# pppKin/rs_ray_toy

Measured on NVIDIA B200. Metric: Mrays/s incoherent closest-hit, higher is better.
Workload: dtype f64 deciding arithmetic (Moller-Trumbore / quadratic), fp32 box culling

## Files before the change

rs_ray_toy_b200/csrc/aggregate.cu:

```cuda
#include <cuda_runtime.h>

#include <chrono>
#include <cmath>
#include <cstdio>
#include <cstdlib>
#include <algorithm>
#include <atomic>
#include <cstring>
#include <thread>
#include <vector>

#include "aggregate.hpp"
#include "bvh_lbvh.hpp"
#include "bvh_pack_plan.hpp"
#include "device_layout.h"
#include "sphere_core.cuh"
#include "tri_screen.h"

namespace rrt {

namespace {

constexpr int kStack = 64;
#ifndef RRT_BLOCK
// ... 140 lines not shown
        *prim_id = (uint32_t)__double2loint(r4.y);
        *kind = (uint32_t)__double2hiint(r4.y);
        *a = {r0.x, r0.y, r1.x};
        *b = {r1.y, r2.x, r2.y};
        *c = {r3.x, r3.y, r4.x};
    }
}

__device__ __noinline__ bool prepare_ray(const AggView& A, D3 o, D3 d, double t_max, float* t_shift, RayF* rf) {
    const double len2 = d.x * d.x + d.y * d.y + d.z * d.z;
    if (!(len2 > 0.0) || !(len2 < 1e300) || !(o.x == o.x) || !(o.y == o.y) || !(o.z == o.z) ||
        fabs(o.x) > 1e300 || fabs(o.y) > 1e300 || fabs(o.z) > 1e300)
        return false;
    double ts = 0.0;
    bool outside = o.x < A.world_lo[0] || o.x > A.world_hi[0] || o.y < A.world_lo[1] || o.y > A.world_hi[1] ||
                   o.z < A.world_lo[2] || o.z > A.world_hi[2];
    if (outside) {
        double t0 = 0.0, t1 = t_max;
        const double oo[3] = {o.x, o.y, o.z}, dd[3] = {d.x, d.y, d.z};
#pragma unroll
        for (int k = 0; k < 3; ++k) {
            if (dd[k] == 0.0) {
                if (oo[k] < A.world_lo[k] || oo[k] > A.world_hi[k]) return false;
                continue;
            }
            double inv = 1.0 / dd[k];
            double ta = (A.world_lo[k] - oo[k]) * inv, tb = (A.world_hi[k] - oo[k]) * inv;
            double tn = fmin(ta, tb), tf = fmax(ta, tb);
            tf *= 1.0 + 1e-12;
            t0 = fmax(t0, tn);
            t1 = fmin(t1, tf);
        }
        if (t0 > t1 * (1.0 + 1e-12) + 1e-300) return false;
        double len = sqrt(d.x * d.x + d.y * d.y + d.z * d.z);
        ts = fmax(0.0, t0 - A.scene_scale / len);
    }
    const float tsf = __double2float_rd(ts);
    ts = (double)tsf;
    *t_shift = tsf;
    double sx = o.x + d.x * ts, sy = o.y + d.y * ts, sz = o.z + d.z * ts;
    const float ix = safe_inv(d.x), iy = safe_inv(d.y), iz = safe_inv(d.z);
    if (A.quantised) {
        rf->idx = A.grid_ext[0] * ix;
        rf->idy = A.grid_ext[1] * iy;
        rf->idz = A.grid_ext[2] * iz;
        rf->oidx = (float)(sx - A.grid_c[0]) * ix;
        rf->oidy = (float)(sy - A.grid_c[1]) * iy;
        rf->oidz = (float)(sz - A.grid_c[2]) * iz;
    } else {
        rf->idx = ix;
        rf->idy = iy;
        rf->idz = iz;
        rf->oidx = (float)sx * ix;
        rf->oidy = (float)sy * iy;
        rf->oidz = (float)sz * iz;
    }
    return true;
}

__device__ __noinline__ bool general_sphere_test(const AggView& A, double index, D3 o, D3 d, double t_far, double* t) {
    const GenSphere& g = static_cast<const GenSphere*>(A.gspheres)[(uint32_t)index];
    V3 p;
    double phi;
    return gen_sphere_hit(g, v3(o.x, o.y, o.z), v3(d.x, d.y, d.z), t_far, t, &p, &phi);
}

template <bool WIDE>
__device__ __noinline__ void hit_params(const AggView& A, uint32_t rec, D3 o, D3 d, double t, double* u, double* v) {
    D3 a, b, c;
    uint32_t pid, kind, inst = 0xFFFFFFFFu;
    load_prim<WIDE>(A.prims, rec, &a, &b, &c, &pid, &kind);
    if (kind == PRIM_TRIANGLE) {
        double tt;
        tri_test(o, d, a, b, c, &tt, u, v);
        return;
    }
    if (kind == PRIM_SPHERE_GENERAL) {
        const GenSphere& g = static_cast<const GenSphere*>(A.gspheres)[(uint32_t)a.x];
        V3 p;
        double phi, tt;
        *u = *v = 0.0;
        if (gen_sphere_hit(g, v3(o.x, o.y, o.z), v3(d.x, d.y, d.z), t, &tt, &p, &phi)) gen_sphere_uv(g, p, phi, u, v);
        return;
    }
    if (!WIDE) inst = static_cast<const PrimRec48*>(A.prims)[rec].words[8];
    else inst = static_cast<const PrimRec96*>(A.prims)[rec].pad[0];
    D3 lo = o, ld = d;
    if (inst != 0xFFFFFFFFu) {
        const double* m = A.inst_w2p + 12 * (size_t)inst;
        lo = {__dadd_rn(__dadd_rn(__dadd_rn(__dmul_rn(m[0], o.x), __dmul_rn(m[1], o.y)), __dmul_rn(m[2], o.z)), m[3]),
              __dadd_rn(__dadd_rn(__dadd_rn(__dmul_rn(m[4], o.x), __dmul_rn(m[5], o.y)), __dmul_rn(m[6], o.z)), m[7]),
              __dadd_rn(__dadd_rn(__dadd_rn(__dmul_rn(m[8], o.x), __dmul_rn(m[9], o.y)), __dmul_rn(m[10], o.z)), m[11])};
        ld = {__dadd_rn(__dadd_rn(__dmul_rn(m[0], d.x), __dmul_rn(m[1], d.y)), __dmul_rn(m[2], d.z)),
              __dadd_rn(__dadd_rn(__dmul_rn(m[4], d.x), __dmul_rn(m[5], d.y)), __dmul_rn(m[6], d.z)),
              __dadd_rn(__dadd_rn(__dmul_rn(m[8], d.x), __dmul_rn(m[9], d.y)), __dmul_rn(m[10], d.z))};
    }
    const double radius = b.x;
    double px = __dadd_rn(lo.x, __dmul_rn(ld.x, t)), py = __dadd_rn(lo.y, __dmul_rn(ld.y, t)),
           pz = __dadd_rn(lo.z, __dmul_rn(ld.z, t));
    if (px == 0.0 && py == 0.0) px = __dmul_rn(1e-5, radius);
    double phi = atan2(py, px);
    const double kPi = 3.14159265358979323846;
    if (phi < 0.0) phi = __dadd_rn(phi, __dmul_rn(2.0, kPi));
    const double phi_max = __dmul_rn(360.0, kPi / 180.0);
    *u = __ddiv_rn(phi, phi_max);
    double cz = __ddiv_rn(pz, radius);
    cz = cz < -1.0 ? -1.0 : (cz > 1.0 ? 1.0 : cz);
    double theta = acos(cz);
    const double theta_min = kPi, theta_max = 0.0;
    *v = __ddiv_rn(__dsub_rn(theta, theta_min), __dsub_rn(theta_max, theta_min));
}

constexpr int32_t kDone = 0x7fffffff;
constexpr int32_t kNoLeaf = 0;
#ifndef RRT_REFILL
#define RRT_REFILL 8
#endif
#ifndef RRT_NODE32
#define RRT_NODE32 1
#endif
#ifndef RRT_STALE_SKIP
#define RRT_STALE_SKIP 0
#endif
#ifndef RRT_STATS
#define RRT_STATS 0
#endif
#ifndef RRT_WALK_MIN
#define RRT_WALK_MIN 12
#endif
#ifndef RRT_PREFETCH_FAR
#define RRT_PREFETCH_FAR 0
#endif
#ifndef RRT_LEAF_MIN
#define RRT_LEAF_MIN 8
#endif
#ifndef RRT_LEAF_TRIPS
#define RRT_LEAF_TRIPS 0
#endif
#ifndef RRT_LEAFQ
#define RRT_LEAFQ 3
#endif
#ifndef RRT_MINBLOCKS
#define RRT_MINBLOCKS 7
#endif
#ifndef RRT_MINBLOCKS_Q
#define RRT_MINBLOCKS_Q 8
#endif
#ifndef RRT_STAGE_TOP
#define RRT_STAGE_TOP 0
#endif
constexpr int kStageTop = RRT_STAGE_TOP;
constexpr int kRefill = RRT_REFILL;
constexpr int kScreenRows = RRT_PRETEST ? 9 : 0;


template <bool ANY, bool WIDE, bool QUANT, bool GEN>
__global__ void __launch_bounds__(kBlock, QUANT ? RRT_MINBLOCKS_Q : RRT_MINBLOCKS) trace_kernel(AggView A, uint64_t n, const rrt_ray* __restrict__ rays,
                                                        rrt_hit* __restrict__ hits, uint8_t* __restrict__ occluded,
                                                        const uint32_t* __restrict__ perm,
                                                        const uint32_t* __restrict__ use_perm,
                                                        unsigned long long* __restrict__ cursor,
                                                        const uint32_t* __restrict__ n_dev, int stack_levels) {
    const unsigned FULL = 0xffffffffu;
    if (n_dev) n = *n_dev;
    const unsigned lane = threadIdx.x & 31u;
    const Node64* __restrict__ nodes = static_cast<const Node64*>(A.nodes);
    const bool permuted = perm != nullptr && (use_perm == nullptr || *use_perm != 0u);

    extern __shared__ int32_t sstack[];
    int32_t* const my_stack = sstack + threadIdx.x;
#if RRT_STALE_SKIP
    float* const my_tstack = reinterpret_cast<float*>(sstack + stack_levels * kBlock) + threadIdx.x;
#define RRT_POP()                                                      \
    do {                                                               \
        --sp;                                                          \
        node = my_stack[sp * kBlock];                                  \
    } while (!ANY && my_tstack[sp * kBlock] > tcull)
#else
#define RRT_POP()                     \
    do {                              \
        --sp;                         \
        node = my_stack[sp * kBlock]; \
    } while (0)
#endif
    float* const my_screen = reinterpret_cast<float*>(sstack + stack_levels * kBlock * (RRT_STALE_SKIP ? 2 : 1)) + threadIdx.x;
#if RRT_STAGE_TOP
    uint4* const s_top = reinterpret_cast<uint4*>(sstack + (stack_levels * (RRT_STALE_SKIP ? 2 : 1) + kScreenRows) * kBlock);
    if (QUANT) {
        const uint4* src = static_cast<const uint4*>(A.nodes);
        const int n_stage = A.n_staged;
        for (int k = threadIdx.x; k < 2 * n_stage; k += kBlock) s_top[k] = __ldg(src + k);
        __syncthreads();
    }
#endif
    int sp = 1;
    int32_t node = kDone;
    int32_t leaf = kNoLeaf;
#if RRT_LEAFQ > 1
    int32_t lq[RRT_LEAFQ - 1];
#pragma unroll
    for (int k = 0; k < RRT_LEAFQ - 1; ++k) lq[k] = kNoLeaf;
#define RRT_PARK()                                         \
    do {                                                   \
        bool placed_ = false;                              \
        if (leaf == kNoLeaf) {                             \
            leaf = node;                                   \
            placed_ = true;                                \
        }                                                  \
        _Pragma("unroll") for (int k_ = 0; k_ < RRT_LEAFQ - 1; ++k_) { \
            if (!placed_ && lq[k_] == kNoLeaf) {           \
                lq[k_] = node;                             \
                placed_ = true;                            \
            }                                              \
        }                                                  \
    } while (0)
#endif
    bool have_ray = false;
    bool exhausted = false;
    uint64_t ray_index = 0;
    D3 o = {0, 0, 0}, d = {0, 0, 0};
    RayF rf = {0, 0, 0, 0, 0, 0};
    uint32_t selx = 0x4105u, sely = 0x4105u, selz = 0x4105u;
    double best_t = 0.0;
    float t_shift = 0.0f, tcull = 0.0f;
    uint32_t best_id = RRT_NO_HIT, best_rec = 0;
    bool found = false;
#if RRT_STATS
    unsigned long long st_trips = 0, st_walk = 0, st_noray = 0, st_drained = 0, st_second = 0, st_ltrips = 0, st_lact = 0;
#endif

    for (;;) {
        const bool finished = have_ray && node == kDone && leaf == kNoLeaf;
        if (finished) {
            if (ANY) {
                occluded[ray_index] = found ? 1 : 0;
            } else {
                double bu = 0.0, bv = 0.0;
                const bool got = best_id != RRT_NO_HIT;
                if (got) hit_params<WIDE>(A, best_rec, o, d, best_t, &bu, &bv);
                double2* hp = reinterpret_cast<double2*>(hits + ray_index);
                double2 w0, w1;
                w0.x = __hiloint2double(0, (int)best_id);
                w0.y = got ? best_t : 0.0;
                w1.x = bu;
                w1.y = bv;
                __stcs(hp, w0);
                __stcs(hp + 1, w1);
            }
            have_ray = false;
        }
        const unsigned idle = __ballot_sync(FULL, !have_ray);
        if (idle != 0u && !exhausted && (__popc(idle) >= kRefill)) {
            const int want = __popc(idle);
            unsigned long long base = 0;
            if (lane == 0) base = atomicAdd(cursor, (unsigned long long)want);
            base = __shfl_sync(FULL, base, 0);
            if (base + (unsigned long long)want >= n) exhausted = true;
            if (!have_ray) {
                const unsigned long long q = base + (unsigned long long)__popc(idle & ((1u << lane) - 1u));
                if (q < n) {
                    ray_index = permuted ? (uint64_t)__ldcs(perm + q) : (uint64_t)q;
                    const double2* rp = reinterpret_cast<const double2*>(rays + ray_index);
                    const double2 q0 = __ldcs(rp), q1 = __ldcs(rp + 1), q2 = __ldcs(rp + 2), q3 = __ldcs(rp + 3);
                    o = {q0.x, q0.y, q1.x};
                    d = {q1.y, q2.x, q2.y};
                    best_t = q3.x;
                    best_id = RRT_NO_HIT;
                    found = false;
                    have_ray = true;
                    sp = 1;
                    my_stack[0] = kDone;
#if RRT_STALE_SKIP
                    my_tstack[0] = -1.0f;
#endif
                    leaf = kNoLeaf;
#if RRT_LEAFQ > 1
#pragma unroll
                    for (int k = 0; k < RRT_LEAFQ - 1; ++k) lq[k] = kNoLeaf;
#endif
                    if (!WIDE && RRT_PRETEST) {
                        const ScreenRay R = make_screen_ray(o.x, o.y, o.z, d.x, d.y, d.z);
                        my_screen[0 * kBlock] = R.ox; my_screen[1 * kBlock] = R.oy; my_screen[2 * kBlock] = R.oz;
                        my_screen[3 * kBlock] = R.dx; my_screen[4 * kBlock] = R.dy; my_screen[5 * kBlock] = R.dz;
                        my_screen[6 * kBlock] = R.mo;
                        my_screen[7 * kBlock] = R.md;
                        my_screen[8 * kBlock] = R.kmd;
                    }
                    const bool live = prepare_ray(A, o, d, best_t, &t_shift, &rf) && !(best_t < 0.0);
                    node = live ? A.root : kDone;
                    tcull = __double2float_ru(best_t - (double)t_shift);
                    if (QUANT && RRT_SIGN_SELECT) {
                        selx = rf.idx < 0.0f ? 0x4325u : 0x4105u;
                        sely = rf.idy < 0.0f ? 0x4325u : 0x4105u;
                        selz = rf.idz < 0.0f ? 0x4325u : 0x4105u;
                    }
                }
            }
        }
        if (__ballot_sync(FULL, have_ray) == 0u) {
            if (exhausted) break;
            continue;
        }

        for (;;) {
#pragma unroll
          for (int step = 0; step < RRT_UNROLL; ++step) {
            const bool walking = node >= 0 && node != kDone;
#if RRT_STATS
            st_trips += 1;
            st_walk += __popc(__ballot_sync(FULL, walking));
            st_noray += __popc(__ballot_sync(FULL, !have_ray));
            st_drained += __popc(__ballot_sync(FULL, have_ray && node == kDone));
            st_second += __popc(__ballot_sync(FULL, have_ray && node < 0));
#endif
            if (walking) {
                int32_t ch_x, ch_y;
                float tn0, tn1;
                bool h0, h1;
                if (QUANT) {
#if RRT_STAGE_TOP
                    F8 v;
                    if (node < A.n_staged) {
                        const uint4 lo = s_top[2 * node], hi = s_top[2 * node + 1];
                        v = F8{__uint_as_float(lo.x), __uint_as_float(lo.y), __uint_as_float(lo.z), __uint_as_float(lo.w),
                               __uint_as_float(hi.x), __uint_as_float(hi.y), __uint_as_float(hi.z), __uint_as_float(hi.w)};
                    } else {
                        v = ldg256(reinterpret_cast<const char*>(A.nodes) + (size_t)node * sizeof(Node32));
                    }
#else
                    const F8 v = ldg256(reinterpret_cast<const char*>(A.nodes) + (size_t)node * sizeof(Node32));
#endif
                    const uint32_t w0 = __float_as_uint(v.a), w1 = __float_as_uint(v.b), w2 = __float_as_uint(v.c);
                    const uint32_t w3 = __float_as_uint(v.d), w4 = __float_as_uint(v.e), w5 = __float_as_uint(v.f);
                    ch_x = __float_as_int(v.g);
                    ch_y = __float_as_int(v.h);
#define RRT_QLO(w) __uint_as_float(__byte_perm((w), 0x3Fu, 0x4105))
#define RRT_QHI(w) __uint_as_float(__byte_perm((w), 0x3Fu, 0x4325))
#if RRT_SIGN_SELECT
                    h0 = slab_q(rf, w0, w1, w2, selx, sely, selz, tcull, &tn0);
                    h1 = slab_q(rf, w3, w4, w5, selx, sely, selz, tcull, &tn1);
#else
                    h0 = slab(rf, RRT_QLO(w0), RRT_QHI(w0), RRT_QLO(w1), RRT_QHI(w1), RRT_QLO(w2), RRT_QHI(w2), tcull, &tn0);
                    h1 = slab(rf, RRT_QLO(w3), RRT_QHI(w3), RRT_QLO(w4), RRT_QHI(w4), RRT_QLO(w5), RRT_QHI(w5), tcull, &tn1);
#endif
                } else {
                    const char* np = reinterpret_cast<const char*>(nodes + node);
                    const F8 lo = ldg256(np);
                    const F8 hi = ldg256(np + 32);
                    ch_x = __float_as_int(hi.e);
                    ch_y = __float_as_int(hi.f);
                    h0 = slab(rf, lo.a, lo.b, lo.c, lo.d, hi.a, hi.b, tcull, &tn0);
                    h1 = slab(rf, lo.e, lo.f, lo.g, lo.h, hi.c, hi.d, tcull, &tn1);
                }
                const bool both = h0 && h1;
                const bool swap = !ANY && (tn1 < tn0);
                const int32_t near_c = swap ? ch_y : ch_x, far_c = swap ? ch_x : ch_y;
                if (both) {
                    my_stack[sp * kBlock] = far_c;
#if RRT_PREFETCH_FAR
                    if (far_c >= 0) {
                        const char* fp = reinterpret_cast<const char*>(A.nodes) + (size_t)far_c * (QUANT ? sizeof(Node32) : sizeof(Node64));
#if RRT_PREFETCH_FAR == 1
                        asm volatile("prefetch.global.L2 [%0];" ::"l"(fp));
#else
                        asm volatile("prefetch.global.L1 [%0];" ::"l"(fp));
#endif
                    }
#endif
#if RRT_STALE_SKIP
                    if (!ANY) my_tstack[sp * kBlock] = swap ? tn0 : tn1;
#endif
                }
                sp += both ? 1 : 0;
                node = both ? near_c : (h0 ? ch_x : ch_y);
                if (!(h0 || h1)) RRT_POP();
            }
#if RRT_LEAFQ > 1
            if (node < 0 && lq[RRT_LEAFQ - 2] == kNoLeaf) {
                RRT_PARK();
                RRT_POP();
            }
#else
            if (node < 0 && leaf == kNoLeaf) {
                leaf = node;
                RRT_POP();
            }
#endif
          }
            if (!__any_sync(FULL, leaf == kNoLeaf && node != kDone)) break;
#if RRT_WALK_MIN > 0
            if (__popc(__ballot_sync(FULL, node >= 0 && node != kDone)) < RRT_WALK_MIN) break;
#endif
        }

#if RRT_LEAF_TRIPS > 0
#pragma unroll 1
        for (int trip = 0; trip < RRT_LEAF_TRIPS && __any_sync(FULL, leaf != kNoLeaf); ++trip) {
#elif RRT_LEAF_MIN > 0
        for (;;) {
            const unsigned with_leaf = __ballot_sync(FULL, leaf != kNoLeaf);
            if (with_leaf == 0u) break;
            if (__popc(with_leaf) < RRT_LEAF_MIN && __any_sync(FULL, node >= 0 && node != kDone)) break;
#else
        while (__any_sync(FULL, leaf != kNoLeaf)) {
#endif
#if RRT_STATS
            st_ltrips += 1;
            st_lact += __popc(__ballot_sync(FULL, leaf != kNoLeaf));
#endif
            if (leaf != kNoLeaf) {
                const uint32_t ref = ~(uint32_t)leaf;
                const uint32_t first = ref >> 3, cnt = (ref & 7u) + 1u;
                uint32_t cand = (1u << cnt) - 1u;
                if (!WIDE && RRT_PRETEST) {
                    ScreenRay R;
                    R.ox = my_screen[0 * kBlock]; R.oy = my_screen[1 * kBlock]; R.oz = my_screen[2 * kBlock];
                    R.dx = my_screen[3 * kBlock]; R.dy = my_screen[4 * kBlock]; R.dz = my_screen[5 * kBlock];
                    R.mo = my_screen[6 * kBlock];
                    R.md = my_screen[7 * kBlock];
                    R.kmd = my_screen[8 * kBlock];
                    R.bt = __double2float_ru(best_t);
                    cand = 0u;
                    for (uint32_t k = 0; k < cnt; ++k) {
                        const float4* p = reinterpret_cast<const float4*>(static_cast<const PrimRec48*>(A.prims) + first + k);
                        const float4 r0 = __ldg(p), r1 = __ldg(p + 1), r2 = __ldg(p + 2);
                        const bool out = __float_as_uint(r2.z) == PRIM_TRIANGLE &&
                                         tri_surely_missed(R, V4f{r0.x, r0.y, r0.z, r0.w}, V4f{r1.x, r1.y, r1.z, r1.w}, V4f{r2.x, r2.y, r2.z, r2.w});
                        cand |= out ? 0u : (1u << k);
                    }
                }
                while (cand != 0u) {
                    const uint32_t k = (uint32_t)__ffs((int)cand) - 1u;
                    cand &= cand - 1u;
                    D3 a, b, c;
                    uint32_t pid, kind;
                    load_prim<WIDE>(A.prims, first + k, &a, &b, &c, &pid, &kind);
                    double t, u, v;
                    bool hit;
                    if (kind == PRIM_TRIANGLE) {
                        hit = tri_test(o, d, a, b, c, &t, &u, &v) && !(t > best_t);
                    } else if (!GEN || kind == PRIM_SPHERE) {
                        hit = sphere_test(o, d, a, b.x, best_t, &t);
                    } else {
                        hit = general_sphere_test(A, a.x, o, d, best_t, &t);
                    }
                    if (hit) {
                        if (ANY) {
                            found = true;
                            break;
                        }
                        if (t < best_t || best_id == RRT_NO_HIT || pid < best_id) {
                            best_t = t;
                            best_id = pid;
                            best_rec = first + k;
                            tcull = __double2float_ru(best_t - (double)t_shift);
                        }
                    }
                }
#if RRT_LEAFQ > 1
                leaf = lq[0];
#pragma unroll
                for (int k = 0; k < RRT_LEAFQ - 2; ++k) lq[k] = lq[k + 1];
                lq[RRT_LEAFQ - 2] = kNoLeaf;
                if (ANY && found) {
                    node = kDone;
                    leaf = kNoLeaf;
#pragma unroll
                    for (int k = 0; k < RRT_LEAFQ - 1; ++k) lq[k] = kNoLeaf;
                } else if (node < 0) {
                    RRT_PARK();
                    RRT_POP();
                }
#else
                leaf = kNoLeaf;
                if (ANY && found) {
                    node = kDone;
                } else if (node < 0) {
                    leaf = node;
                    RRT_POP();
                }
#endif
            }
        }
    }
#if RRT_STATS
    if (lane == 0) {
        atomicAdd(cursor + 2, st_trips);
        atomicAdd(cursor + 3, st_walk);
        atomicAdd(cursor + 4, st_noray);
        atomicAdd(cursor + 5, st_drained);
        atomicAdd(cursor + 6, st_second);
        atomicAdd(cursor + 7, st_ltrips);
        atomicAdd(cursor + 8, st_lact);
    }
#endif
}

#ifndef RRT_SORTBITS
#define RRT_SORTBITS 7
#endif
constexpr int kSortBits = RRT_SORTBITS;
constexpr uint32_t kSortBins = (1u << (3 * kSortBits)) * 8u;

__device__ __forceinline__ uint32_t spread3(uint32_t x) {
    x = (x | (x << 16)) & 0x030000FFu;
    x = (x | (x << 8)) & 0x0300F00Fu;
    x = (x | (x << 4)) & 0x030C30C3u;
    x = (x | (x << 2)) & 0x09249249u;
    return x;
}

__device__ __forceinline__ uint32_t ray_key(const AggView& A, const rrt_ray* r, int bits) {
    const double2* rp = reinterpret_cast<const double2*>(r);
    const double2 q0 = __ldg(rp), q1 = __ldg(rp + 1), q2 = __ldg(rp + 2);
    const double o[3] = {q0.x, q0.y, q1.x};
    const double dd[3] = {q1.y, q2.x, q2.y};
    uint32_t c[3];
#pragma unroll
    for (int k = 0; k < 3; ++k) {
        double ext = A.world_hi[k] - A.world_lo[k];
        double f = ext > 0.0 ? (o[k] - A.world_lo[k]) / ext : 0.0;
        f = f < 0.0 ? 0.0 : (f > 1.0 ? 1.0 : f);
        if (!(f == f)) f = 0.0;
        uint32_t q = (uint32_t)(f * (double)(1u << bits));
        c[k] = q >= (1u << bits) ? (1u << bits) - 1u : q;
    }
    const uint32_t cell = spread3(c[0]) | (spread3(c[1]) << 1) | (spread3(c[2]) << 2);
    const uint32_t oct = (dd[0] < 0.0 ? 1u : 0u) | (dd[1] < 0.0 ? 2u : 0u) | (dd[2] < 0.0 ? 4u : 0u);
    if (A.sort_mode == 0) return cell;
    if (A.sort_mode == 2) return (oct << (3 * bits)) | cell;
    return (cell << 3) | oct;
}

__global__ void __launch_bounds__(256) sort_count_kernel(AggView A, uint64_t n, const rrt_ray* __restrict__ rays,
                                                          uint32_t* __restrict__ bins, uint32_t* __restrict__ key_out,
                                                          uint32_t* __restrict__ rank_out,
                                                          const uint32_t* __restrict__ n_dev, int bits) {
    if (n_dev) n = *n_dev;
    const unsigned lane = threadIdx.x & 31u;
    for (uint64_t base = (uint64_t)blockIdx.x * blockDim.x; base < n; base += (uint64_t)gridDim.x * blockDim.x) {
        const uint64_t i = base + threadIdx.x;
        const bool valid = i < n;
        const uint32_t key = valid ? ray_key(A, rays + i, bits) : 0xFFFFFFFFu;
        const unsigned peers = __match_any_sync(0xffffffffu, key);
        const int leader = __ffs(peers) - 1;
        uint32_t first = 0;
        if (valid && (int)lane == leader) first = atomicAdd(bins + key, (uint32_t)__popc(peers));
        first = __shfl_sync(0xffffffffu, first, leader);
        if (valid) {
            key_out[i] = key;
            rank_out[i] = first + (uint32_t)__popc(peers & ((1u << lane) - 1u));
        }
    }
}

constexpr int kScanBlock = 1024;
__global__ void __launch_bounds__(kScanBlock) scan_block_kernel(uint32_t* __restrict__ bins, uint32_t nbins,
                                                                 uint32_t* __restrict__ block_sums,
                                                                 uint32_t* __restrict__ max_bin) {
    __shared__ uint32_t warp_sums[32];
    const uint32_t i = blockIdx.x * kScanBlock + threadIdx.x;
    const uint32_t v = i < nbins ? bins[i] : 0u;
    const unsigned lane = threadIdx.x & 31u, warp = threadIdx.x >> 5;
    uint32_t x = v;
#pragma unroll
    for (int off = 1; off < 32; off <<= 1) {
        uint32_t y = __shfl_up_sync(0xffffffffu, x, off);
        if ((int)lane >= off) x += y;
    }
    uint32_t m = v;
#pragma unroll
    for (int off = 16; off > 0; off >>= 1) m = max(m, __shfl_xor_sync(0xffffffffu, m, off));
    if (lane == 31) warp_sums[warp] = x;
    if (lane == 0 && m > 0) atomicMax(max_bin, m);
    __syncthreads();
    if (warp == 0) {
        uint32_t w = warp_sums[lane];
#pragma unroll
        for (int off = 1; off < 32; off <<= 1) {
            uint32_t y = __shfl_up_sync(0xffffffffu, w, off);
            if ((int)lane >= off) w += y;
        }
        warp_sums[lane] = w;
    }
    __syncthreads();
    const uint32_t incl = x + (warp > 0 ? warp_sums[warp - 1] : 0u);
    if (i < nbins) bins[i] = incl - v;
    if (threadIdx.x == kScanBlock - 1) block_sums[blockIdx.x] = incl;
}
__global__ void __launch_bounds__(kScanBlock) scan_sums_kernel(uint32_t* __restrict__ block_sums, uint32_t nblocks,
                                                                const uint32_t* __restrict__ max_bin, uint64_t n,
                                                                uint32_t* __restrict__ use_perm,
                                                                const uint32_t* __restrict__ n_dev) {
    if (n_dev) n = *n_dev;
    __shared__ uint32_t warp_sums[32];
    __shared__ uint32_t carry;
    if (threadIdx.x == 0) {
        carry = 0;
        const uint32_t mb = *max_bin;
        *use_perm = (((uint64_t)mb * 64u > n && mb >= 4096u) || n < 4096u) ? 0u : 1u;
    }
    __syncthreads();
    const unsigned lane = threadIdx.x & 31u, warp = threadIdx.x >> 5;
    for (uint32_t base = 0; base < nblocks; base += kScanBlock) {
        const uint32_t i = base + threadIdx.x;
        const uint32_t v = i < nblocks ? block_sums[i] : 0u;
        uint32_t x = v;
#pragma unroll
// ... 371 lines not shown
                    const Bvh2Node& nd = tree.nodes[plan[i].tn];
                    Node64 o;
                    std::memset(&o, 0, sizeof(o));
                    set_child(o, 0, tree.nodes[nd.left].box);
                    set_child(o, 1, tree.nodes[nd.right].box);
                    o.child0 = plan[i].child0;
                    o.child1 = plan[i].child1;
                    nodes[i] = o;
                }
            });
            parallel_ranges(leaves.size(), [&](size_t i0, size_t i1) {
                for (size_t i = i0; i < i1; ++i) {
                    const Bvh2Node& nd = tree.nodes[leaves[i].tn];
                    for (uint32_t k = 0; k < nd.count; ++k) make_record(tree.order[nd.first + k], (size_t)leaves[i].first + k);
                }
            });
        }
    }

    int n_staged = 0;
    if (kStageTop > 0 && quantise && !on_device_ok && nodes.size() > (size_t)kStageTop) {
        std::vector<uint32_t> top;
        top.push_back(0);
        for (size_t h = 0; h < top.size() && top.size() < (size_t)kStageTop; ++h) {
            const Node64& nd = nodes[top[h]];
            if (nd.child0 >= 0 && top.size() < (size_t)kStageTop) top.push_back((uint32_t)nd.child0);
            if (nd.child1 >= 0 && top.size() < (size_t)kStageTop) top.push_back((uint32_t)nd.child1);
        }
        std::vector<int32_t> new_index(nodes.size(), -1);
        for (size_t k = 0; k < top.size(); ++k) new_index[top[k]] = (int32_t)k;
        int32_t next = (int32_t)top.size();
        for (size_t i = 0; i < nodes.size(); ++i)
            if (new_index[i] < 0) new_index[i] = next++;
        std::vector<Node64> moved(nodes.size());
        for (size_t i = 0; i < nodes.size(); ++i) {
            Node64 nd = nodes[i];
            if (nd.child0 >= 0) nd.child0 = new_index[nd.child0];
            if (nd.child1 >= 0) nd.child1 = new_index[nd.child1];
            moved[new_index[i]] = nd;
        }
        nodes.swap(moved);
        n_staged = (int)top.size();
    }
    view_.n_staged = n_staged;
    std::vector<Node32> nodes32;
    if (quantise && !on_device_ok) {
        nodes32.resize(nodes.size());
        auto quant = [&](double plane, int k, bool upper) -> uint32_t {
            const double cell = (double)grid_ext[k] / 32768.0;
            const double margin = (double)grid_ext[k] * std::ldexp(1.0, -19);
            double q = upper ? std::ceil((plane + margin - grid_lo[k]) / cell) : std::floor((plane - margin - grid_lo[k]) / cell);
            if (q < 0.0) q = 0.0;
            if (q > 32767.0) q = 32767.0;
            return 0x8000u | (uint32_t)q;
        };
        parallel_ranges(nodes.size(), [&](size_t i0, size_t i1) {
        for (size_t i = i0; i < i1; ++i) {
            const Node64& s = nodes[i];
            Node32 o;
            o.p[0] = quant(s.c0_lox, 0, false) | (quant(s.c0_hix, 0, true) << 16);
            o.p[1] = quant(s.c0_loy, 1, false) | (quant(s.c0_hiy, 1, true) << 16);
            o.p[2] = quant(s.c0_loz, 2, false) | (quant(s.c0_hiz, 2, true) << 16);
            o.p[3] = quant(s.c1_lox, 0, false) | (quant(s.c1_hix, 0, true) << 16);
            o.p[4] = quant(s.c1_loy, 1, false) | (quant(s.c1_hiy, 1, true) << 16);
            o.p[5] = quant(s.c1_loz, 2, false) | (quant(s.c1_hiz, 2, true) << 16);
            o.child0 = s.child0;
            o.child1 = s.child1;
            nodes32[i] = o;
        }
        });
    }
    lap("pack nodes + records");
    RRT_CUDA(cudaSetDevice(device));
    const size_t node_bytes = on_device_ok ? lb.node_bytes : (quantise ? nodes32.size() * sizeof(Node32) : nodes.size() * sizeof(Node64));
    const void* node_src = quantise ? (const void*)nodes32.data() : (const void*)nodes.data();
    size_t prim_bytes = wide ? n * sizeof(PrimRec96) : n * sizeof(PrimRec48);
    if (on_device_ok) {
        d_nodes_ = lb.d_nodes;
    } else {
        RRT_CUDA(cudaMalloc(&d_nodes_, node_bytes));
        RRT_CUDA(cudaMemcpy(d_nodes_, node_src, node_bytes, cudaMemcpyHostToDevice));
    }
    RRT_CUDA(cudaMalloc(&d_prims_, prim_bytes));
    RRT_CUDA(cudaMemcpy(d_prims_, wide ? (const void*)rec96.get() : (const void*)rec48.get(), prim_bytes,
                        cudaMemcpyHostToDevice));
    bool has_spheres = false;
    for (const Primitive& pr : scene.prims) has_spheres |= pr.kind == SHAPE_SPHERE;
    if (has_spheres && !scene.instances.empty()) {
        std::vector<double> w2p(12 * scene.instances.size());
        for (size_t i = 0; i < scene.instances.size(); ++i)
            for (int r = 0; r < 3; ++r)
                for (int c = 0; c < 4; ++c) w2p[12 * i + 4 * r + c] = scene.instances[i].inv.m[r][c];
        RRT_CUDA(cudaMalloc(&d_inst_, w2p.size() * sizeof(double)));
        RRT_CUDA(cudaMemcpy(d_inst_, w2p.data(), w2p.size() * sizeof(double), cudaMemcpyHostToDevice));
    }
    if (!gspheres.empty()) {
        RRT_CUDA(cudaMalloc(&d_gspheres_, gspheres.size() * sizeof(GenSphere)));
        RRT_CUDA(cudaMemcpy(d_gspheres_, gspheres.data(), gspheres.size() * sizeof(GenSphere), cudaMemcpyHostToDevice));
    }
    view_.gspheres = d_gspheres_;
    lap("upload");
    l2_window_bytes_ = 0;
    {
        const char* e = std::getenv("RRT_L2_PERSIST");
        int max_persist = 0, max_window = 0;
        cudaDeviceGetAttribute(&max_persist, cudaDevAttrMaxPersistingL2CacheSize, device);
        cudaDeviceGetAttribute(&max_window, cudaDevAttrMaxAccessPolicyWindowSize, device);
        if (e && atoi(e) != 0 && max_persist > 0 && max_window > 0) {
            const size_t want = std::min<size_t>(node_bytes, (size_t)max_window);
            cudaDeviceSetLimit(cudaLimitPersistingL2CacheSize, std::min<size_t>((size_t)max_persist, want));
            l2_window_bytes_ = want;
            l2_hit_ratio_ = (float)std::min(1.0, (double)std::min<size_t>((size_t)max_persist, want) / (double)want);
        }
    }
    view_.inst_w2p = static_cast<const double*>(d_inst_);
    view_.has_spheres = has_spheres ? 1 : 0;
    view_.nodes = d_nodes_;
    view_.prims = d_prims_;
    for (int k = 0; k < 3; ++k) {
        view_.world_lo[k] = world_box.lo[k] - delta;
        view_.world_hi[k] = world_box.hi[k] + delta;
    }
    view_.scene_scale = scale;
    for (int k = 0; k < 3; ++k) {
        view_.grid_c[k] = grid_c[k];
        view_.grid_ext[k] = grid_ext[k];
    }
    view_.quantised = quantise ? 1 : 0;
    view_.root = 0;
    view_.wide = wide ? 1 : 0;
    view_.sort_mode = 0;
    if (const char* e = std::getenv("RRT_SORT_MODE")) view_.sort_mode = atoi(e);
    if (const char* e = std::getenv("RRT_SORT")) sort_rays_ = atoi(e) != 0;
    stats_.n_nodes = on_device_ok ? lb.n_nodes : nodes.size();
    stats_.tree_device_usec = on_device_ok ? (uint64_t)(lb.device_ms * 1000.0f) : 0;
    stats_.n_leaves = tree.n_leaves;
    stats_.max_depth = tree.max_depth;
    stats_.device_bytes = node_bytes + prim_bytes;
    stats_.n_records = n;
    stats_.wide_records = wide;
    stats_.n_prims = n;
    stats_.build_usec =
        (uint64_t)std::chrono::duration_cast<std::chrono::microseconds>(std::chrono::steady_clock::now() - t_start).count();
    stack_levels_ = (int)tree.max_depth + 2;
    node_bytes_ = node_bytes;
    prim_bytes_ = prim_bytes;
    inst_bytes_ = d_inst_ ? 12 * scene.instances.size() * sizeof(double) : 0;
    gsphere_bytes_ = gspheres.size() * sizeof(GenSphere);
    configure_kernels(quantise);
    return RRT_OK;
}

void DeviceAggregate::configure_kernels(bool quantise) {
    const size_t smem = ((size_t)stack_levels_ * (RRT_STALE_SKIP ? 2 : 1) + kScreenRows) * kBlock * sizeof(int32_t) + (size_t)kStageTop * sizeof(Node32);
    int carve = (int)(((quantise ? RRT_MINBLOCKS_Q : RRT_MINBLOCKS) * smem * 100 + 227 * 1024 - 1) / (227 * 1024)) + 2;
    if (carve > 100) carve = 100;
    for (auto fn : {(const void*)trace_kernel<false, false, false, false>, (const void*)trace_kernel<false, true, false, false>,
                    (const void*)trace_kernel<true, false, false, false>, (const void*)trace_kernel<true, true, false, false>,
                    (const void*)trace_kernel<false, false, true, false>, (const void*)trace_kernel<false, true, true, false>,
                    (const void*)trace_kernel<true, false, true, false>, (const void*)trace_kernel<true, true, true, false>,
                    (const void*)trace_kernel<false, false, false, true>, (const void*)trace_kernel<false, true, false, true>,
                    (const void*)trace_kernel<true, false, false, true>, (const void*)trace_kernel<true, true, false, true>,
                    (const void*)trace_kernel<false, false, true, true>, (const void*)trace_kernel<false, true, true, true>,
                    (const void*)trace_kernel<true, false, true, true>, (const void*)trace_kernel<true, true, true, true>}) {
        cudaFuncSetAttribute(fn, cudaFuncAttributeMaxDynamicSharedMemorySize, (int)smem);
        cudaFuncSetAttribute(fn, cudaFuncAttributePreferredSharedMemoryCarveout, carve);
    }
}

namespace {
struct BlobHeader {
    uint64_t magic, version;
    AggView view;
    AggregateStats stats;
    int32_t stack_levels, sort_rays;
    uint64_t node_bytes, prim_bytes, inst_bytes, gsphere_bytes;
};
constexpr uint64_t kBlobMagic = 0x3130454552545252ull;
}

int DeviceAggregate::export_blob(void* buffer, uint64_t capacity, uint64_t* bytes, std::string* err) const {
    const uint64_t total = sizeof(BlobHeader) + node_bytes_ + prim_bytes_ + inst_bytes_ + gsphere_bytes_;
    *bytes = total;
    if (!buffer) return RRT_OK;
    if (capacity < total) {
        if (err) *err = "export_blob: buffer too small";
        return RRT_ERR_INVALID;
    }
    BlobHeader h{};
    h.magic = kBlobMagic;
    h.version = 1;
    h.view = view_;
    h.view.nodes = h.view.prims = h.view.gspheres = nullptr;
    h.view.inst_w2p = nullptr;
    h.stats = stats_;
    h.stack_levels = stack_levels_;
    h.sort_rays = sort_rays_ ? 1 : 0;
    h.node_bytes = node_bytes_;
    h.prim_bytes = prim_bytes_;
    h.inst_bytes = inst_bytes_;
    h.gsphere_bytes = gsphere_bytes_;
    char* out = static_cast<char*>(buffer);
    std::memcpy(out, &h, sizeof(h));
    out += sizeof(h);
    RRT_CUDA(cudaSetDevice(device_));
    RRT_CUDA(cudaMemcpy(out, d_nodes_, node_bytes_, cudaMemcpyDeviceToHost));
    out += node_bytes_;
    RRT_CUDA(cudaMemcpy(out, d_prims_, prim_bytes_, cudaMemcpyDeviceToHost));
    out += prim_bytes_;
    if (inst_bytes_) RRT_CUDA(cudaMemcpy(out, d_inst_, inst_bytes_, cudaMemcpyDeviceToHost));
    out += inst_bytes_;
    if (gsphere_bytes_) RRT_CUDA(cudaMemcpy(out, d_gspheres_, gsphere_bytes_, cudaMemcpyDeviceToHost));
    return RRT_OK;
}

int DeviceAggregate::import_blob(int device, const void* blob, uint64_t bytes, uint64_t n_prims_expected, std::string* err) {
    auto t_start = std::chrono::steady_clock::now();
    BlobHeader h;
    if (bytes < sizeof(h)) {
        if (err) *err = "import_blob: truncated";
        return RRT_ERR_INVALID;
    }
    std::memcpy(&h, blob, sizeof(h));
    if (h.magic != kBlobMagic || h.version != 1 ||
        bytes != sizeof(h) + h.node_bytes + h.prim_bytes + h.inst_bytes + h.gsphere_bytes) {
        if (err) *err = "import_blob: not a tree exported by this library version";
        return RRT_ERR_INVALID;
    }
    if (h.stats.n_prims != n_prims_expected) {
        if (err) *err = "import_blob: the tree was built over " + std::to_string(h.stats.n_prims) + " primitives, the scene holds " + std::to_string(n_prims_expected);
        return RRT_ERR_INVALID;
    }
    if (h.stack_levels < 2 || h.stack_levels > kStack) {
        if (err) *err = "import_blob: bad stack depth";
        return RRT_ERR_INVALID;
    }
    device_ = device;
    RRT_CUDA(cudaSetDevice(device));
    const char* in = static_cast<const char*>(blob) + sizeof(h);
    RRT_CUDA(cudaMalloc(&d_nodes_, h.node_bytes));
    RRT_CUDA(cudaMemcpy(d_nodes_, in, h.node_bytes, cudaMemcpyHostToDevice));
    in += h.node_bytes;
    RRT_CUDA(cudaMalloc(&d_prims_, h.prim_bytes));
    RRT_CUDA(cudaMemcpy(d_prims_, in, h.prim_bytes, cudaMemcpyHostToDevice));
    in += h.prim_bytes;
    if (h.inst_bytes) {
        RRT_CUDA(cudaMalloc(&d_inst_, h.inst_bytes));
        RRT_CUDA(cudaMemcpy(d_inst_, in, h.inst_bytes, cudaMemcpyHostToDevice));
    }
    in += h.inst_bytes;
    if (h.gsphere_bytes) {
        RRT_CUDA(cudaMalloc(&d_gspheres_, h.gsphere_bytes));
        RRT_CUDA(cudaMemcpy(d_gspheres_, in, h.gsphere_bytes, cudaMemcpyHostToDevice));
    }
    view_ = h.view;
    view_.nodes = d_nodes_;
    view_.prims = d_prims_;
    view_.inst_w2p = static_cast<const double*>(d_inst_);
    view_.gspheres = d_gspheres_;
    stats_ = h.stats;
    stack_levels_ = h.stack_levels;
    sort_rays_ = h.sort_rays != 0;
    node_bytes_ = h.node_bytes;
    prim_bytes_ = h.prim_bytes;
    inst_bytes_ = h.inst_bytes;
    gsphere_bytes_ = h.gsphere_bytes;
    stats_.build_usec =
        (uint64_t)std::chrono::duration_cast<std::chrono::microseconds>(std::chrono::steady_clock::now() - t_start).count();
    configure_kernels(view_.quantised != 0);
    return RRT_OK;
}

int DeviceAggregate::ensure_workspace(Workspace& w, uint64_t n, std::string* err) const {
    if (!w.d_small) {
        RRT_CUDA(cudaMalloc(&w.d_bins, (size_t)kSortBins * sizeof(uint32_t)));
        RRT_CUDA(cudaMalloc(&w.d_block_sums, (size_t)(kSortBins / kScanBlock) * sizeof(uint32_t)));
        RRT_CUDA(cudaMalloc(&w.d_small, 128));
        RRT_CUDA(cudaEventCreateWithFlags(&w.last_use, cudaEventDisableTiming));
        int dev = 0, sms = 0;
        RRT_CUDA(cudaGetDevice(&dev));
        RRT_CUDA(cudaDeviceGetAttribute(&sms, cudaDevAttrMultiProcessorCount, dev));
        w.n_sms = sms;
    }
    if (n > w.capacity) {
        if (w.d_key) cudaFree(w.d_key);
        if (w.d_rank) cudaFree(w.d_rank);
        if (w.d_perm) cudaFree(w.d_perm);
        w.d_key = w.d_rank = w.d_perm = nullptr;
        w.capacity = 0;
        RRT_CUDA(cudaMalloc(&w.d_key, n * sizeof(uint32_t)));
        RRT_CUDA(cudaMalloc(&w.d_rank, n * sizeof(uint32_t)));
        RRT_CUDA(cudaMalloc(&w.d_perm, n * sizeof(uint32_t)));
        w.capacity = n;
    }
    return RRT_OK;
}

template <bool ANY>
int DeviceAggregate::trace(uint64_t n, const rrt_ray* d_rays, rrt_hit* d_hits, uint8_t* d_occ, void* stream,
                           std::string* err, int* launches, const uint32_t* n_dev) const {
    if (n == 0) return RRT_OK;
    if (n >= (1ull << 32)) {
        if (err) *err = "batch too large for one call (2^32 rays)";
        return RRT_ERR_INVALID;
    }
    cudaStream_t s = static_cast<cudaStream_t>(stream);
    std::lock_guard<std::mutex> lock(ws_mutex_);
    Workspace& w = (ws_.count(stream) || ws_.size() < kMaxWorkspaces) ? ws_[stream] : ws_.begin()->second;
    int rc = ensure_workspace(w, n, err);
    if (rc != RRT_OK) return rc;
    if (w.used && w.last_stream != stream) RRT_CUDA(cudaStreamWaitEvent(s, w.last_use, 0));
    uint32_t* small = static_cast<uint32_t*>(w.d_small);
    RRT_CUDA(cudaMemsetAsync(small, 0, 128, s));
    const bool sorting = sort_rays_ && n >= 4096;
    int count = 0;
    if (sorting) {
        int bits = kSortBits;
        while (bits > 4 && (1ull << (3 * bits)) > 2 * n) --bits;
        const uint32_t nbins = (1u << (3 * bits)) * (view_.sort_mode == 0 ? 1u : 8u);
        RRT_CUDA(cudaMemsetAsync(w.d_bins, 0, (size_t)nbins * sizeof(uint32_t), s));
        const unsigned sb = (unsigned)std::min<uint64_t>((n + 255) / 256, (uint64_t)w.n_sms * 16u);
        sort_count_kernel<<<sb, 256, 0, s>>>(view_, n, d_rays, w.d_bins, w.d_key, w.d_rank, n_dev, bits);
        scan_block_kernel<<<nbins / kScanBlock, kScanBlock, 0, s>>>(w.d_bins, nbins, w.d_block_sums, small + 2);
        scan_sums_kernel<<<1, kScanBlock, 0, s>>>(w.d_block_sums, nbins / kScanBlock, small + 2, n, small + 3, n_dev);
        sort_scatter_kernel<<<sb, 256, 0, s>>>(n, w.d_bins, w.d_block_sums, w.d_key, w.d_rank, small + 3, w.d_perm,
                                               n_dev);
        count += 4;
    }
    auto kernel = view_.gspheres != nullptr
                      ? (view_.quantised ? (view_.wide ? trace_kernel<ANY, true, true, true> : trace_kernel<ANY, false, true, true>)
                                         : (view_.wide ? trace_kernel<ANY, true, false, true> : trace_kernel<ANY, false, false, true>))
                      : (view_.quantised ? (view_.wide ? trace_kernel<ANY, true, true, false> : trace_kernel<ANY, false, true, false>)
                                         : (view_.wide ? trace_kernel<ANY, true, false, false> : trace_kernel<ANY, false, false, false>));
    const size_t smem = ((size_t)stack_levels_ * (RRT_STALE_SKIP ? 2 : 1) + kScreenRows) * kBlock * sizeof(int32_t) + (size_t)kStageTop * sizeof(Node32);
    int per_sm = 0;
    RRT_CUDA(cudaOccupancyMaxActiveBlocksPerMultiprocessor(&per_sm, kernel, kBlock, smem));
    if (per_sm < 1) per_sm = 1;
    uint64_t blocks = (uint64_t)w.n_sms * (uint64_t)per_sm;
    const uint64_t needed = (n + kBlock - 1) / kBlock;
    if (blocks > needed) blocks = needed;
    if (l2_window_bytes_ && w.window_stream != s) {
        cudaStreamAttrValue attr{};
        attr.accessPolicyWindow.base_ptr = d_nodes_;
        attr.accessPolicyWindow.num_bytes = l2_window_bytes_;
        attr.accessPolicyWindow.hitRatio = l2_hit_ratio_;
        attr.accessPolicyWindow.hitProp = cudaAccessPropertyPersisting;
        attr.accessPolicyWindow.missProp = cudaAccessPropertyStreaming;
        cudaStreamSetAttribute(s, cudaStreamAttributeAccessPolicyWindow, &attr);
        w.window_stream = s;
    }
    kernel<<<(unsigned)blocks, kBlock, smem, s>>>(view_, n, d_rays, d_hits, d_occ, sorting ? w.d_perm : nullptr,
                                               sorting ? small + 3 : nullptr,
                                               reinterpret_cast<unsigned long long*>(small), n_dev, stack_levels_);
    count += 1;
    RRT_CUDA(cudaGetLastError());
#if RRT_STATS
    {
        unsigned long long h[16];
        RRT_CUDA(cudaStreamSynchronize(s));
        RRT_CUDA(cudaMemcpy(h, small, 128, cudaMemcpyDeviceToHost));
        if (n >= (1u << 20))
            fprintf(stderr, "RRT_STATS any=%d n=%llu interior trips %llu: walking %.2f no-ray %.2f drained %.2f at-2nd-leaf %.2f | leaf trips %llu: active %.2f\n",
                    (int)ANY, (unsigned long long)n, h[2], (double)h[3] / h[2], (double)h[4] / h[2], (double)h[5] / h[2],
                    (double)h[6] / h[2], h[7], (double)h[8] / (h[7] ? h[7] : 1));
    }
#endif
    RRT_CUDA(cudaEventRecord(w.last_use, s));
    w.used = true;
    w.last_stream = stream;
    if (launches) *launches = count;
    return RRT_OK;
}

int DeviceAggregate::closest_hit(uint64_t n, const rrt_ray* d_rays, rrt_hit* d_hits, void* stream, std::string* err,
                                 int* launches) const {
    return trace<false>(n, d_rays, d_hits, nullptr, stream, err, launches, nullptr);
}
int DeviceAggregate::closest_hit_indirect(uint64_t capacity, const uint32_t* d_count, const rrt_ray* d_rays,
                                          rrt_hit* d_hits, void* stream, std::string* err, int* launches) const {
    return trace<false>(capacity, d_rays, d_hits, nullptr, stream, err, launches, d_count);
}
int DeviceAggregate::any_hit_indirect(uint64_t capacity, const uint32_t* d_count, const rrt_ray* d_rays,
                                      uint8_t* d_occluded, void* stream, std::string* err, int* launches) const {
    return trace<true>(capacity, d_rays, nullptr, d_occluded, stream, err, launches, d_count);
}

int DeviceAggregate::any_hit(uint64_t n, const rrt_ray* d_rays, uint8_t* d_occluded, void* stream, std::string* err,
                             int* launches) const {
    return trace<true>(n, d_rays, nullptr, d_occluded, stream, err, launches, nullptr);
}

}
```

Baseline: 1486.

## Spill ray origin/direction and cold per-ray state to shared memory

Moves the ray's double-precision origin and direction, ray index, best record and t_shift out of registers into per-thread shared-memory slots, reloading them only in leaf tests and at hit finalisation. It also turns the stack index into a pointer that advances by the block stride and redoes the shared-memory layout and carveout calculation. The aim is to cut register pressure so more warps fit per SM under the launch bounds, at the cost of extra shared-memory traffic on every leaf visit and more shared memory per block.

```diff
diff --git a/rs_ray_toy_b200/csrc/aggregate.cu b/rs_ray_toy_b200/csrc/aggregate.cu
--- a/rs_ray_toy_b200/csrc/aggregate.cu
+++ b/rs_ray_toy_b200/csrc/aggregate.cu
@@ -316,6 +316,27 @@
 constexpr int kStageTop = RRT_STAGE_TOP;
 constexpr int kRefill = RRT_REFILL;
 constexpr int kScreenRows = RRT_PRETEST ? 9 : 0;
+#ifndef RRT_RAY_SMEM
+#define RRT_RAY_SMEM 1
+#endif
+constexpr int kRayRows = RRT_RAY_SMEM ? 6 : 0;
+constexpr int kWordRows = 3;
+
+struct TraceSmem {
+    size_t ray, word, screen, stack, tstack, top, bytes;
+};
+__host__ __device__ constexpr size_t align_up(size_t v, size_t a) { return (v + a - 1) / a * a; }
+__host__ __device__ constexpr TraceSmem trace_smem(int stack_levels) {
+    TraceSmem s{};
+    s.ray = 0;
+    s.word = s.ray + (size_t)kRayRows * kBlock * sizeof(double);
+    s.screen = s.word + (size_t)kWordRows * kBlock * sizeof(uint32_t);
+    s.stack = s.screen + (size_t)kScreenRows * kBlock * sizeof(float);
+    s.tstack = s.stack + (size_t)stack_levels * kBlock * sizeof(int32_t);
+    s.top = align_up(s.tstack + (RRT_STALE_SKIP ? (size_t)stack_levels * kBlock * sizeof(float) : 0), 16);
+    s.bytes = s.top + (size_t)kStageTop * sizeof(Node32);
+    return s;
+}
 
 
 template <bool ANY, bool WIDE, bool QUANT, bool GEN>
@@ -331,25 +352,41 @@
     const Node64* __restrict__ nodes = static_cast<const Node64*>(A.nodes);
     const bool permuted = perm != nullptr && (use_perm == nullptr || *use_perm != 0u);
 
-    extern __shared__ int32_t sstack[];
-    int32_t* const my_stack = sstack + threadIdx.x;
+    extern __shared__ __align__(16) char smem[];
+    constexpr TraceSmem L = trace_smem(0);
+    double* const my_ray = reinterpret_cast<double*>(smem + L.ray) + threadIdx.x;
+    uint32_t* const my_ray_index = reinterpret_cast<uint32_t*>(smem + L.word) + threadIdx.x;
+    uint32_t* const my_best_rec = my_ray_index + kBlock;
+    float* const my_t_shift = reinterpret_cast<float*>(my_ray_index + 2 * kBlock);
+    auto load_ray = [&](D3* o, D3* d) {
+        if (RRT_RAY_SMEM) {
+            *o = {my_ray[0 * kBlock], my_ray[1 * kBlock], my_ray[2 * kBlock]};
+            *d = {my_ray[3 * kBlock], my_ray[4 * kBlock], my_ray[5 * kBlock]};
+        } else {
+            const double2* rp = reinterpret_cast<const double2*>(rays + *my_ray_index);
+            const double2 q0 = __ldg(rp), q1 = __ldg(rp + 1), q2 = __ldg(rp + 2);
+            *o = {q0.x, q0.y, q1.x};
+            *d = {q1.y, q2.x, q2.y};
+        }
+    };
+    int32_t* const my_stack = reinterpret_cast<int32_t*>(smem + L.stack) + threadIdx.x;
 #if RRT_STALE_SKIP
-    float* const my_tstack = reinterpret_cast<float*>(sstack + stack_levels * kBlock) + threadIdx.x;
-#define RRT_POP()                                                      \
-    do {                                                               \
-        --sp;                                                          \
-        node = my_stack[sp * kBlock];                                  \
-    } while (!ANY && my_tstack[sp * kBlock] > tcull)
+    const int tstack_delta = stack_levels * kBlock;
+#define RRT_POP()                                                                  \
+    do {                                                                           \
+        sp -= kBlock;                                                              \
+        node = *sp;                                                                \
+    } while (!ANY && *reinterpret_cast<const float*>(sp + tstack_delta) > tcull)
 #else
-#define RRT_POP()                     \
-    do {                              \
-        --sp;                         \
-        node = my_stack[sp * kBlock]; \
+#define RRT_POP()          \
+    do {                   \
+        sp -= kBlock;      \
+        node = *sp;        \
     } while (0)
 #endif
-    float* const my_screen = reinterpret_cast<float*>(sstack + stack_levels * kBlock * (RRT_STALE_SKIP ? 2 : 1)) + threadIdx.x;
+    float* const my_screen = reinterpret_cast<float*>(smem + L.screen) + threadIdx.x;
 #if RRT_STAGE_TOP
-    uint4* const s_top = reinterpret_cast<uint4*>(sstack + (stack_levels * (RRT_STALE_SKIP ? 2 : 1) + kScreenRows) * kBlock);
+    uint4* const s_top = reinterpret_cast<uint4*>(smem + trace_smem(stack_levels).top);
     if (QUANT) {
         const uint4* src = static_cast<const uint4*>(A.nodes);
         const int n_stage = A.n_staged;
@@ -357,7 +394,7 @@
         __syncthreads();
     }
 #endif
-    int sp = 1;
+    int32_t* sp = my_stack + kBlock;
     int32_t node = kDone;
     int32_t leaf = kNoLeaf;
 #if RRT_LEAFQ > 1
@@ -381,13 +418,11 @@
 #endif
     bool have_ray = false;
     bool exhausted = false;
-    uint64_t ray_index = 0;
-    D3 o = {0, 0, 0}, d = {0, 0, 0};
     RayF rf = {0, 0, 0, 0, 0, 0};
     uint32_t selx = 0x4105u, sely = 0x4105u, selz = 0x4105u;
     double best_t = 0.0;
-    float t_shift = 0.0f, tcull = 0.0f;
-    uint32_t best_id = RRT_NO_HIT, best_rec = 0;
+    float tcull = 0.0f;
+    uint32_t best_id = RRT_NO_HIT;
     bool found = false;
 #if RRT_STATS
     unsigned long long st_trips = 0, st_walk = 0, st_noray = 0, st_drained = 0, st_second = 0, st_ltrips = 0, st_lact = 0;
@@ -396,12 +431,17 @@
     for (;;) {
         const bool finished = have_ray && node == kDone && leaf == kNoLeaf;
         if (finished) {
+            const uint32_t ray_index = *my_ray_index;
             if (ANY) {
                 occluded[ray_index] = found ? 1 : 0;
             } else {
                 double bu = 0.0, bv = 0.0;
                 const bool got = best_id != RRT_NO_HIT;
-                if (got) hit_params<WIDE>(A, best_rec, o, d, best_t, &bu, &bv);
+                if (got) {
+                    D3 o, d;
+                    load_ray(&o, &d);
+                    hit_params<WIDE>(A, *my_best_rec, o, d, best_t, &bu, &bv);
+                }
                 double2* hp = reinterpret_cast<double2*>(hits + ray_index);
                 double2 w0, w1;
                 w0.x = __hiloint2double(0, (int)best_id);
@@ -423,19 +463,23 @@
             if (!have_ray) {
                 const unsigned long long q = base + (unsigned long long)__popc(idle & ((1u << lane) - 1u));
                 if (q < n) {
-                    ray_index = permuted ? (uint64_t)__ldcs(perm + q) : (uint64_t)q;
+                    const uint32_t ray_index = permuted ? __ldcs(perm + q) : (uint32_t)q;
+                    *my_ray_index = ray_index;
                     const double2* rp = reinterpret_cast<const double2*>(rays + ray_index);
                     const double2 q0 = __ldcs(rp), q1 = __ldcs(rp + 1), q2 = __ldcs(rp + 2), q3 = __ldcs(rp + 3);
-                    o = {q0.x, q0.y, q1.x};
-                    d = {q1.y, q2.x, q2.y};
+                    const D3 o = {q0.x, q0.y, q1.x}, d = {q1.y, q2.x, q2.y};
+                    if (RRT_RAY_SMEM) {
+                        my_ray[0 * kBlock] = o.x; my_ray[1 * kBlock] = o.y; my_ray[2 * kBlock] = o.z;
+                        my_ray[3 * kBlock] = d.x; my_ray[4 * kBlock] = d.y; my_ray[5 * kBlock] = d.z;
+                    }
                     best_t = q3.x;
                     best_id = RRT_NO_HIT;
                     found = false;
                     have_ray = true;
-                    sp = 1;
+                    sp = my_stack + kBlock;
                     my_stack[0] = kDone;
 #if RRT_STALE_SKIP
-                    my_tstack[0] = -1.0f;
+                    *reinterpret_cast<float*>(my_stack + tstack_delta) = -1.0f;
 #endif
                     leaf = kNoLeaf;
 #if RRT_LEAFQ > 1
@@ -450,7 +494,9 @@
                         my_screen[7 * kBlock] = R.md;
                         my_screen[8 * kBlock] = R.kmd;
                     }
+                    float t_shift = 0.0f;
                     const bool live = prepare_ray(A, o, d, best_t, &t_shift, &rf) && !(best_t < 0.0);
+                    *my_t_shift = t_shift;
                     node = live ? A.root : kDone;
                     tcull = __double2float_ru(best_t - (double)t_shift);
                     if (QUANT && RRT_SIGN_SELECT) {
@@ -520,7 +566,7 @@
                 const bool swap = !ANY && (tn1 < tn0);
                 const int32_t near_c = swap ? ch_y : ch_x, far_c = swap ? ch_x : ch_y;
                 if (both) {
-                    my_stack[sp * kBlock] = far_c;
+                    *sp = far_c;
 #if RRT_PREFETCH_FAR
                     if (far_c >= 0) {
                         const char* fp = reinterpret_cast<const char*>(A.nodes) + (size_t)far_c * (QUANT ? sizeof(Node32) : sizeof(Node64));
@@ -532,10 +578,10 @@
                     }
 #endif
 #if RRT_STALE_SKIP
-                    if (!ANY) my_tstack[sp * kBlock] = swap ? tn0 : tn1;
+                    if (!ANY) *reinterpret_cast<float*>(sp + tstack_delta) = swap ? tn0 : tn1;
 #endif
                 }
-                sp += both ? 1 : 0;
+                sp += both ? kBlock : 0;
                 node = both ? near_c : (h0 ? ch_x : ch_y);
                 if (!(h0 || h1)) RRT_POP();
             }
@@ -593,6 +639,8 @@
                         cand |= out ? 0u : (1u << k);
                     }
                 }
+                D3 o, d;
+                load_ray(&o, &d);
                 while (cand != 0u) {
                     const uint32_t k = (uint32_t)__ffs((int)cand) - 1u;
                     cand &= cand - 1u;
@@ -616,8 +664,8 @@
                         if (t < best_t || best_id == RRT_NO_HIT || pid < best_id) {
                             best_t = t;
                             best_id = pid;
-                            best_rec = first + k;
-                            tcull = __double2float_ru(best_t - (double)t_shift);
+                            *my_best_rec = first + k;
+                            tcull = __double2float_ru(best_t - (double)*my_t_shift);
                         }
                     }
                 }
@@ -1295,8 +1343,10 @@
 }
 
 void DeviceAggregate::configure_kernels(bool quantise) {
-    const size_t smem = ((size_t)stack_levels_ * (RRT_STALE_SKIP ? 2 : 1) + kScreenRows) * kBlock * sizeof(int32_t) + (size_t)kStageTop * sizeof(Node32);
-    int carve = (int)(((quantise ? RRT_MINBLOCKS_Q : RRT_MINBLOCKS) * smem * 100 + 227 * 1024 - 1) / (227 * 1024)) + 2;
+    const size_t smem = trace_smem(stack_levels_).bytes;
+    const size_t per_sm = (size_t)(quantise ? RRT_MINBLOCKS_Q : RRT_MINBLOCKS) * (smem + 1024);
+    const size_t max_smem = 228 * 1024;
+    int carve = (int)((per_sm * 100 + max_smem - 1) / max_smem);
     if (carve > 100) carve = 100;
     for (auto fn : {(const void*)trace_kernel<false, false, false, false>, (const void*)trace_kernel<false, true, false, false>,
                     (const void*)trace_kernel<true, false, false, false>, (const void*)trace_kernel<true, true, false, false>,
@@ -1475,7 +1525,7 @@
                                          : (view_.wide ? trace_kernel<ANY, true, false, true> : trace_kernel<ANY, false, false, true>))
                       : (view_.quantised ? (view_.wide ? trace_kernel<ANY, true, true, false> : trace_kernel<ANY, false, true, false>)
                                          : (view_.wide ? trace_kernel<ANY, true, false, false> : trace_kernel<ANY, false, false, false>));
-    const size_t smem = ((size_t)stack_levels_ * (RRT_STALE_SKIP ? 2 : 1) + kScreenRows) * kBlock * sizeof(int32_t) + (size_t)kStageTop * sizeof(Node32);
+    const size_t smem = trace_smem(stack_levels_).bytes;
     int per_sm = 0;
     RRT_CUDA(cudaOccupancyMaxActiveBlocksPerMultiprocessor(&per_sm, kernel, kBlock, smem));
     if (per_sm < 1) per_sm = 1;
```

Result: faster. 1512, median of 6 (+1.8%).
